# alibaba/TorchEasyRec

Measured on NVIDIA H100. Metric: samples/sec (DLRM-Criteo synth, train step fwd+bwd+optimizer), higher is better.
Workload: dtype f32

## Files before the change

torcheasyrec_b200/csrc/tzk_tower.cu:

```cuda
#include <cstdlib>

#include "tzk_common.cuh"

#include "tzk_launch.cuh"
#include "tzk_tower_bwd2.cuh"
#include "tzk_tower_tail.cuh"

using namespace tzk;

namespace {
constexpr int kTM = 128;

__device__ __forceinline__ int odd(int v) { return v | 1; }
constexpr int kNW = kTM / 32;
constexpr int kLU = 16;

__device__ __forceinline__ void load_tile(float* dst, int S, const float* __restrict__ src, int64_t ld,
                                          const float* __restrict__ mask, int64_t ld_m, int rows, int C) {
  const int warp = threadIdx.x >> 5, lane = threadIdx.x & 31;
  for (int r0 = warp; r0 < rows; r0 += kNW * kLU) {
    float v[kLU][2], m[kLU][2];
#pragma unroll
    for (int q = 0; q < kLU; ++q) {
      const int r = r0 + q * kNW;
// ... 262 lines not shown
  if ((threadIdx.x & 31) == 0) red[threadIdx.x >> 5] = acc;
  __syncthreads();
  if (threadIdx.x == 0) {
    float s = 0.f;
    for (int k = 0; k < kBceThreads / 32; ++k) s += red[k];
    partial[blockIdx.x] = s;
  }
}
__global__ void __launch_bounds__(256)
bce_final_kernel(const float* __restrict__ partial, int n, float inv_m, float* __restrict__ loss) {
  __shared__ float red[256];
  float s = 0.f;
  for (int i = threadIdx.x; i < n; i += 256) s += partial[i];
  red[threadIdx.x] = s;
  __syncthreads();
  for (int d = 128; d >= 1; d >>= 1) {
    if (threadIdx.x < d) red[threadIdx.x] += red[threadIdx.x + d];
    __syncthreads();
  }
  if (threadIdx.x == 0) loss[0] = red[0] * inv_m;
}
}

static int small_linear_check(const char* who, int64_t M, int32_t K, int32_t N) {
  TZK_REQUIRE(M >= 0, "%s: negative M", who);
  TZK_REQUIRE(K >= 1 && K <= 64 && N >= 1 && N <= 64, "%s: K=%d, N=%d outside [1,64]", who, K, N);
  return 0;
}

extern "C" int tzk_small_linear_fwd(const float* x, int64_t ld_x, const float* w, const float* bias, int64_t M,
                                    int32_t K, int32_t N, int32_t relu, float* y, int64_t ld_y,
                                    tzk_stream_t stream) {
  int rc = small_linear_check("small_linear_fwd", M, K, N);
  if (rc) return rc;
  if (M == 0) return 0;
  TZK_REQUIRE(x && w && y, "small_linear_fwd: NULL argument");
  TZK_REQUIRE(ld_x >= K && ld_y >= N, "small_linear_fwd: leading dimension smaller than the row");
  const int NP = pad_pow(N, 4);
  {
    const size_t smem_r = ((size_t)K * NP + NP) * sizeof(float);
    const bool vec = (K % 4 == 0) && (ld_x % 4 == 0) && ((uintptr_t)x % 16 == 0);
    const int64_t blocks = ceil_div64(M, kRowThreads);
    const int grid_r = (int)(blocks < kSmCountH100 * 16 ? blocks : kSmCountH100 * 16);
#define TZK_SLR(NP_)                                                                                                \
  do {                                                                                                              \
    if (vec)                                                                                                        \
      small_linear_fwd_rows_kernel<NP_, true><<<grid_r, kRowThreads, smem_r, as_stream(stream)>>>(                  \
          x, ld_x, w, bias, M, K, N, relu, y, ld_y);                                                                \
    else                                                                                                            \
      small_linear_fwd_rows_kernel<NP_, false><<<grid_r, kRowThreads, smem_r, as_stream(stream)>>>(                 \
          x, ld_x, w, bias, M, K, N, relu, y, ld_y);                                                                \
  } while (0)
    switch (NP) {
      case 4: TZK_SLR(4); break;
      case 16: TZK_SLR(16); break;
      case 32: TZK_SLR(32); break;
      default: TZK_SLR(64); break;
    }
#undef TZK_SLR
    TZK_CHECK_LAUNCH("small_linear_fwd_rows_kernel");
  }
  return 0;
}

static bool use_bwd2(int K, int N) {
  const char* e = getenv("TZK_SMALL_LINEAR_BWD");
  return !(e && e[0] == '1') && tzk_bwd2::supported(K, N);
}

extern "C" size_t tzk_small_linear_bwd_workspace_bytes(int64_t M, int32_t K, int32_t N) {
  const size_t v1 = (size_t)bwd_grid(M) * ((size_t)(N < 1 ? 1 : N) * (K < 1 ? 1 : K) + (N < 1 ? 1 : N)) * sizeof(float);
  const size_t v2 = tzk_bwd2::supported(K, N) ? tzk_bwd2::workspace_bytes(M < 1 ? 1 : M, K, N) : 0;
  return v1 > v2 ? v1 : v2;
}

extern "C" int tzk_small_linear_bwd(const float* x, int64_t ld_x, const float* w, const float* y, int64_t ld_y,
                                    const float* dy, int64_t ld_dy, int64_t M, int32_t K, int32_t N, int32_t relu,
                                    float* dx, int64_t ld_dx, float* dw, float* db, void* workspace,
                                    size_t workspace_bytes, tzk_stream_t stream) {
  int rc = small_linear_check("small_linear_bwd", M, K, N);
  if (rc) return rc;
  TZK_REQUIRE(M >= 1, "small_linear_bwd: empty batch");
  TZK_REQUIRE(x && w && dy && dw && (!relu || y), "small_linear_bwd: NULL argument");
  TZK_REQUIRE(ld_x >= K && ld_dy >= N && (!relu || ld_y >= N) && (!dx || ld_dx >= K),
              "small_linear_bwd: leading dimension smaller than the row");
  TZK_REQUIRE(workspace && workspace_bytes >= tzk_small_linear_bwd_workspace_bytes(M, K, N),
              "small_linear_bwd: workspace too small");
  if (use_bwd2(K, N)) {
    rc = tzk_bwd2::run(x, ld_x, w, y, ld_y, dy, ld_dy, M, K, N, relu, dx, ld_dx, dw, db, workspace, workspace_bytes,
                       as_stream(stream));
    TZK_REQUIRE(rc == 0, "small_linear_bwd: tzk_bwd2::run failed with code %d", rc);
    return 0;
  }
  const int KP = pad_pow(K, 16), NP = pad_pow(N, 4);
  const int grid = bwd_grid(M);
  const size_t smem = ((size_t)N * KP + (size_t)kTM * (K | 1) + (size_t)kTM * (N | 1)) * sizeof(float);
  float* partial = static_cast<float*>(workspace);
  cudaStream_t st = as_stream(stream);
#define TZK_SLB(KP_, NP_)                                                                                          \
  do {                                                                                                             \
    if (smem > 48 * 1024)                                                                                          \
      cudaFuncSetAttribute(small_linear_bwd_kernel<KP_, NP_>, cudaFuncAttributeMaxDynamicSharedMemorySize,         \
                           (int)smem);                                                                             \
    small_linear_bwd_kernel<KP_, NP_><<<grid, kTM, smem, st>>>(x, ld_x, w, y, ld_y, dy, ld_dy, M, K, N, relu, dx,   \
                                                               ld_dx, partial);                                    \
  } while (0)
#define TZK_SLB_N(KP_)                      \
  switch (NP) {                             \
    case 4: TZK_SLB(KP_, 4); break;         \
    case 16: TZK_SLB(KP_, 16); break;       \
    case 32: TZK_SLB(KP_, 32); break;       \
    default: TZK_SLB(KP_, 64); break;       \
  }
  switch (KP) {
    case 16: TZK_SLB_N(16) break;
    case 32: TZK_SLB_N(32) break;
    default: TZK_SLB_N(64) break;
  }
#undef TZK_SLB_N
#undef TZK_SLB
  TZK_CHECK_LAUNCH("small_linear_bwd_kernel");
  const int total = N * K + N;
  small_linear_reduce_kernel<<<(total + 31) / 32, 256, 0, st>>>(partial, grid, N * K, N, dw, db);
  TZK_CHECK_LAUNCH("small_linear_reduce_kernel");
  return 0;
}

extern "C" size_t tzk_bce_logits_workspace_bytes(int64_t M) {
  return (size_t)ceil_div64(M < 1 ? 1 : M, kBceThreads * kBcePerThread) * sizeof(float);
}

extern "C" int tzk_bce_logits_fwd_bwd(const float* logits, const float* labels, int64_t M, float* loss,
                                      float* dlogits, void* workspace, size_t workspace_bytes,
                                      tzk_stream_t stream) {
  TZK_REQUIRE(M >= 1, "bce_logits: empty batch");
  TZK_REQUIRE(logits && labels && loss, "bce_logits: NULL argument");
  TZK_REQUIRE(workspace && workspace_bytes >= tzk_bce_logits_workspace_bytes(M), "bce_logits: workspace too small");
  const int64_t nb = ceil_div64(M, kBceThreads * kBcePerThread);
  TZK_REQUIRE(nb < ((int64_t)1 << 31), "bce_logits: batch too large");
  float* partial = static_cast<float*>(workspace);
  cudaStream_t st = as_stream(stream);
  const float inv_m = 1.0f / (float)M;
  bce_fwd_bwd_kernel<<<(unsigned)nb, kBceThreads, 0, st>>>(logits, labels, M, inv_m, dlogits, partial);
  TZK_CHECK_LAUNCH("bce_fwd_bwd_kernel");
  bce_final_kernel<<<1, 256, 0, st>>>(partial, (int)nb, inv_m, loss);
  TZK_CHECK_LAUNCH("bce_final_kernel");
  return 0;
}

extern "C" size_t tzk_tower_tail_bce_workspace_bytes(int64_t M, int32_t K, int32_t N) {
  return tzk_tail::supported(K, N) ? tzk_tail::workspace_bytes(M < 1 ? 1 : M, K, N) : 0;
}

extern "C" int tzk_tower_tail_bce(const float* y1, int64_t ld_y, const float* w1, const float* b1, const float* w2,
                                  const float* b2, const float* labels, int64_t M, int32_t K, int32_t N, float* logits,
                                  float* dy1, int64_t ld_dy, float* colsum, float* out, void* workspace,
                                  size_t workspace_bytes, tzk_stream_t stream) {
  TZK_REQUIRE(M >= 1, "tower_tail_bce: empty batch");
  TZK_REQUIRE(tzk_tail::supported(K, N), "tower_tail_bce: K=%d, N=%d must be in [1, 64]", K, N);
  TZK_REQUIRE(y1 && w1 && w2 && labels && logits && dy1 && out, "tower_tail_bce: NULL argument");
  TZK_REQUIRE(ld_y >= K && ld_dy >= K, "tower_tail_bce: leading dimension smaller than the row");
  TZK_REQUIRE(workspace && workspace_bytes >= tzk_tower_tail_bce_workspace_bytes(M, K, N),
              "tower_tail_bce: workspace too small");
  const int rc = tzk_tail::run(y1, ld_y, w1, b1, w2, b2, labels, M, K, N, logits, dy1, ld_dy, out, workspace,
                               workspace_bytes, as_stream(stream), colsum != nullptr);
  TZK_REQUIRE(rc == 0, "tower_tail_bce: tzk_tail::run failed with code %d", rc);
  if (colsum) {
    colsum_final(static_cast<const float*>(workspace) + tzk_tail::colsum_offset(M, K, N), tzk_tail::tiles(M), K, colsum,
                 as_stream(stream));
    TZK_CHECK_LAUNCH("colsum_final_kernel");
  }
  return 0;
}
```

torcheasyrec_b200/csrc/tzk_tower_tail.cuh:

```cuda
#pragma once
#include <stdint.h>

namespace tzk_tail {
constexpr int kRows = 128;
constexpr int kMaxCtas = 132 * 4;

__device__ __forceinline__ bool aligned16(const void* p) { return (reinterpret_cast<uintptr_t>(p) & 15) == 0; }

inline int out_len(int K, int N) { return N * K + 2 * N + 2; }
inline int grid_for(int64_t M) {
  const int64_t t = (M + kRows - 1) / kRows;
  return (int)(t < 1 ? 1 : (t < kMaxCtas ? t : kMaxCtas));
}
inline int64_t tiles(int64_t M) { return (M + kRows - 1) / kRows; }
inline size_t colsum_offset(int64_t M, int K, int N) { return (size_t)grid_for(M) * out_len(K, N); }
inline size_t workspace_bytes(int64_t M, int K, int N) {
  return (colsum_offset(M, K, N) + (size_t)tiles(M) * K) * sizeof(float);
}
inline size_t smem_bytes(int KP, int NP, bool mask) {
  return ((size_t)NP * KP + 2 * NP + (size_t)(mask ? 2 : 1) * kRows * (KP + 4) + 2 * (size_t)kRows * NP + 2 * kRows) *
         sizeof(float);
}

template <int KP, int NP, bool kMask>
__global__ void __launch_bounds__(kRows)
tower_tail_bce_kernel(const float* __restrict__ y1, int64_t ld_y, const float* __restrict__ w1,
                      const float* __restrict__ b1, const float* __restrict__ w2, const float* __restrict__ b2,
                      const float* __restrict__ labels, int64_t M, int K, int N, float inv_m, int rows_per_cta,
                      float* __restrict__ logits, float* __restrict__ dy1, int64_t ld_dy, float* __restrict__ partial,
                      float* __restrict__ zsum) {
  constexpr int R = kRows, KC = KP / 4, NC = NP / 4, XS = KP + 4;
  constexpr int NB = (KC * NC + R - 1) / R;
  TZK_DYN_SMEM(float, sm);
  float* Ws = sm;
  float* b1s = Ws + NP * KP;
  float* w2s = b1s + NP;
  float* Xs = w2s + NP;
  float* Dh = Xs + R * XS;
  float* Hg = Dh + R * NP;
  float* Dz = Hg + R * NP;
  float* Ls = Dz + R;
  float* Zs = Ls + R;
  const int tid = threadIdx.x;
  for (int i = tid; i < NP * KP; i += R) {
    const int n = i / KP, k = i - n * KP;
    Ws[i] = (n < N && k < K) ? __ldg(w1 + (int64_t)n * K + k) : 0.f;
  }
  for (int n = tid; n < NP; n += R) {
    b1s[n] = (n < N && b1) ? __ldg(b1 + n) : 0.f;
    w2s[n] = n < N ? __ldg(w2 + n) : 0.f;
  }
  const float b2v = b2 ? __ldg(b2) : 0.f;
  const bool vin = (K & 3) == 0 && (ld_y & 3) == 0 && aligned16(y1);
  const bool vout = (K & 3) == 0 && (ld_dy & 3) == 0 && aligned16(dy1);
  float acc[NB][4][4], accv = 0.f, accw = 0.f, accz = 0.f, accl = 0.f;
#pragma unroll
  for (int q = 0; q < NB; ++q)
#pragma unroll
    for (int i = 0; i < 4; ++i)
#pragma unroll
      for (int j = 0; j < 4; ++j) acc[q][i][j] = 0.f;
  const int64_t row_begin = (int64_t)blockIdx.x * rows_per_cta;
  const int64_t row_end = row_begin + rows_per_cta < M ? row_begin + rows_per_cta : M;
  __syncthreads();
  for (int64_t t0 = row_begin; t0 < row_end; t0 += R) {
    const int64_t row = t0 + tid;
    const bool live = row < row_end;
    float* xr = Xs + tid * XS;
#pragma unroll
    for (int c = 0; c < KC; ++c) {
      float4 v = make_float4(0.f, 0.f, 0.f, 0.f);
      if (live && 4 * c < K) {
        const float* p = y1 + row * ld_y + 4 * c;
        if (vin) {
          v = *reinterpret_cast<const float4*>(p);
        } else {
          v.x = __ldg(p);
          if (4 * c + 1 < K) v.y = __ldg(p + 1);
          if (4 * c + 2 < K) v.z = __ldg(p + 2);
          if (4 * c + 3 < K) v.w = __ldg(p + 3);
        }
      }
      *reinterpret_cast<float4*>(xr + 4 * c) = v;
    }
    float h[NP];
#pragma unroll
    for (int n = 0; n < NP; ++n) h[n] = b1s[n];
#pragma unroll 2
    for (int c = 0; c < KC; ++c) {
      const float4 x4 = *reinterpret_cast<const float4*>(xr + 4 * c);
#pragma unroll
      for (int n = 0; n < NP; ++n) {
        const float4 w4 = *reinterpret_cast<const float4*>(Ws + n * KP + 4 * c);
        h[n] = fmaf(x4.x, w4.x, h[n]);
        h[n] = fmaf(x4.y, w4.y, h[n]);
        h[n] = fmaf(x4.z, w4.z, h[n]);
        h[n] = fmaf(x4.w, w4.w, h[n]);
      }
    }
    float z = b2v;
#pragma unroll
    for (int n = 0; n < NP; ++n) {
      h[n] = h[n] > 0.f ? h[n] : 0.f;
      z = fmaf(h[n], w2s[n], z);
    }
    float dz = 0.f, lt = 0.f;
    if (live) {
      const float y = __ldg(labels + row);
      const float e = expf(-fabsf(z));
      lt = fmaxf(z, 0.f) - z * y + log1pf(e);
      const float sig = z >= 0.f ? 1.f / (1.f + e) : e / (1.f + e);
      dz = (sig - y) * inv_m;
      logits[row] = z;
    }
    Dz[tid] = dz;
    Ls[tid] = lt;
#pragma unroll
    for (int n = 0; n < NP; ++n) {
      Hg[tid * NP + n] = dz * h[n];
      h[n] = h[n] > 0.f ? dz * w2s[n] : 0.f;
      Dh[tid * NP + n] = h[n];
    }
#pragma unroll 2
    for (int c = 0; c < KC; ++c) {
      float4 a = make_float4(0.f, 0.f, 0.f, 0.f);
#pragma unroll
      for (int n = 0; n < NP; ++n) {
        const float4 w4 = *reinterpret_cast<const float4*>(Ws + n * KP + 4 * c);
        a.x = fmaf(h[n], w4.x, a.x);
        a.y = fmaf(h[n], w4.y, a.y);
        a.z = fmaf(h[n], w4.z, a.z);
        a.w = fmaf(h[n], w4.w, a.w);
      }
      if constexpr (kMask) {
        const float4 y4 = *reinterpret_cast<const float4*>(xr + 4 * c);
        a.x = y4.x > 0.f ? a.x : 0.f;
        a.y = y4.y > 0.f ? a.y : 0.f;
        a.z = y4.z > 0.f ? a.z : 0.f;
        a.w = y4.w > 0.f ? a.w : 0.f;
        *reinterpret_cast<float4*>(Zs + tid * XS + 4 * c) = a;
      }
      if (live && 4 * c < K) {
        float* p = dy1 + row * ld_dy + 4 * c;
        if (vout) {
          *reinterpret_cast<float4*>(p) = a;
        } else {
          p[0] = a.x;
          if (4 * c + 1 < K) p[1] = a.y;
          if (4 * c + 2 < K) p[2] = a.z;
          if (4 * c + 3 < K) p[3] = a.w;
        }
      }
    }
    __syncthreads();
#pragma unroll
    for (int q = 0; q < NB; ++q) {
      const int blk = tid + q * R;
      if (blk < KC * NC) {
        const int tn = blk / KC, tk = blk - tn * KC;
        const float* dp = Dh + 4 * tn;
        const float* xp = Xs + 4 * tk;
#pragma unroll 4
        for (int r = 0; r < R; ++r) {
          const float4 a4 = *reinterpret_cast<const float4*>(dp + r * NP);
          const float4 b4 = *reinterpret_cast<const float4*>(xp + r * XS);
          const float a[4] = {a4.x, a4.y, a4.z, a4.w}, b[4] = {b4.x, b4.y, b4.z, b4.w};
#pragma unroll
          for (int i = 0; i < 4; ++i)
#pragma unroll
            for (int j = 0; j < 4; ++j) acc[q][i][j] = fmaf(a[i], b[j], acc[q][i][j]);
        }
      }
    }
    if (tid < NP) {
      for (int r = 0; r < R; ++r) {
        accv += Dh[r * NP + tid];
        accw += Hg[r * NP + tid];
      }
    }
    if (tid == 0) {
      for (int r = 0; r < R; ++r) {
        accz += Dz[r];
        accl += Ls[r];
      }
    }
    if constexpr (kMask) {
      const int c = tid - (R - KP);
      if (c >= 0 && c < K) {
        float s[4] = {0.f, 0.f, 0.f, 0.f};
#pragma unroll 4
        for (int r = 0; r < R; r += 4)
#pragma unroll
          for (int j = 0; j < 4; ++j) s[j] += Zs[(r + j) * XS + c];
        float v = 0.f;
#pragma unroll
        for (int j = 0; j < 4; ++j) v += s[j];
        zsum[t0 / R * K + c] = v;
      }
    }
    __syncthreads();
  }
  float* out = partial + (int64_t)blockIdx.x * (N * K + 2 * N + 2);
#pragma unroll
  for (int q = 0; q < NB; ++q) {
    const int blk = tid + q * R;
    if (blk < KC * NC) {
      const int tn = blk / KC, tk = blk - tn * KC;
#pragma unroll
      for (int i = 0; i < 4; ++i)
#pragma unroll
        for (int j = 0; j < 4; ++j)
          if (4 * tn + i < N && 4 * tk + j < K) out[(4 * tn + i) * K + 4 * tk + j] = acc[q][i][j];
    }
  }
  if (tid < N) {
    out[N * K + tid] = accv;
    out[N * K + N + tid] = accw;
  }
  if (tid == 0) {
    out[N * K + 2 * N] = accz;
    out[N * K + 2 * N + 1] = accl;
  }
}

__global__ void __launch_bounds__(256)
tower_tail_reduce_kernel(const float* __restrict__ partial, int n_parts, int len, float inv_m, float* __restrict__ out) {
  __shared__ float red[8][32];
  const int o = threadIdx.x & 31, g = threadIdx.x >> 5;
  const int i = blockIdx.x * 32 + o;
  float s = 0.f;
  if (i < len)
    for (int c = g; c < n_parts; c += 8) s += partial[(int64_t)c * len + i];
  red[g][o] = s;
  __syncthreads();
  if (g == 0 && i < len) {
    float r = 0.f;
#pragma unroll
    for (int k = 0; k < 8; ++k) r += red[k][o];
    out[i] = i == len - 1 ? r * inv_m : r;
  }
}

inline bool supported(int K, int N) { return K >= 1 && N >= 1 && K <= 64 && N <= 64; }

inline int run(const float* y1, int64_t ld_y, const float* w1, const float* b1, const float* w2, const float* b2,
               const float* labels, int64_t M, int32_t K, int32_t N, float* logits, float* dy1, int64_t ld_dy,
               float* out, void* workspace, size_t workspace_bytes_, cudaStream_t st, bool mask = false) {
  if (M < 1 || !supported(K, N) || !y1 || !w1 || !w2 || !labels || !logits || !dy1 || !out || ld_y < K || ld_dy < K) return 1;
  if (workspace_bytes_ < workspace_bytes(M, K, N)) return 2;
  const int KP = K <= 16 ? 16 : (K <= 32 ? 32 : 64);
  const int NP = N <= 16 ? 16 : (N <= 32 ? 32 : 64);
  const int grid = grid_for(M);
  int rows_per_cta = (int)((M + grid - 1) / grid);
  rows_per_cta = (rows_per_cta + kRows - 1) / kRows * kRows;
  const float inv_m = 1.0f / (float)M;
  const size_t smem = smem_bytes(KP, NP, mask);
  float* partial = static_cast<float*>(workspace);
  float* zsum = partial + colsum_offset(M, K, N);
#ifdef TZK_CPU_SHIM
#define TZK_TAIL_ATTR(KP_, NP_, MASK_)
#else
#define TZK_TAIL_ATTR(KP_, NP_, MASK_)                                                                                \
  if (smem > 48 * 1024)                                                                                               \
    cudaFuncSetAttribute(tower_tail_bce_kernel<KP_, NP_, MASK_>, cudaFuncAttributeMaxDynamicSharedMemorySize, (int)smem);
#endif
#define TZK_TAIL(KP_, NP_, MASK_)                                                                                     \
  do {                                                                                                                \
    TZK_TAIL_ATTR(KP_, NP_, MASK_)                                                                                    \
    TZK_LAUNCH((tower_tail_bce_kernel<KP_, NP_, MASK_>), grid, kRows, smem, st, y1, ld_y, w1, b1, w2, b2, labels, M,  \
               K, N, inv_m, rows_per_cta, logits, dy1, ld_dy, partial, zsum);                                         \
  } while (0)
#define TZK_TAIL_N(KP_, MASK_)                                                                                        \
  do {                                                                                                                \
    if (NP == 16) TZK_TAIL(KP_, 16, MASK_);                                                                           \
    else if (NP == 32) TZK_TAIL(KP_, 32, MASK_);                                                                      \
    else TZK_TAIL(KP_, 64, MASK_);                                                                                    \
  } while (0)
#define TZK_TAIL_K(MASK_)                                                                                             \
  do {                                                                                                                \
    if (KP == 16) TZK_TAIL_N(16, MASK_);                                                                              \
    else if (KP == 32) TZK_TAIL_N(32, MASK_);                                                                         \
    else TZK_TAIL_N(64, MASK_);                                                                                       \
  } while (0)
  if (mask) TZK_TAIL_K(true);
  else TZK_TAIL_K(false);
#undef TZK_TAIL_K
#undef TZK_TAIL_N
#undef TZK_TAIL
#undef TZK_TAIL_ATTR
  if (cudaGetLastError() != cudaSuccess) return 3;
  const int len = out_len(K, N);
  TZK_LAUNCH((tower_tail_reduce_kernel), (len + 31) / 32, 256, 0, st, partial, grid, len, inv_m, out);
  return cudaGetLastError() == cudaSuccess ? 0 : 3;
}
}
```

torcheasyrec_b200/kernels.py:

```python

import ctypes
import math
import os
import threading
from dataclasses import dataclass
from typing import List, Optional, Sequence, Tuple

import torch

from ._lib import TzkError, check, lib

POOL_SUM, POOL_MEAN = 0, 1
OPT_SGD, OPT_ADAGRAD, OPT_ROWWISE_ADAGRAD, OPT_ADAM, OPT_PARTIAL_ROWWISE_ADAM = 0, 1, 2, 3, 4
OPT_LAMB, OPT_PARTIAL_ROWWISE_LAMB, OPT_LARS_SGD = 5, 6, 7
WD_NONE, WD_L2, WD_DECOUPLE = 0, 1, 2
LARS_ETA = 0.001
OPT_ACCUM_OUT = 100


@dataclass
class FeatureLayout:

    w_off: List[int]
    rows: List[int]
# ... 794 lines not shown
        d_sparse = torch.empty((B, 416), dtype=torch.float32, device=sparse.device)
        check(self._lib.tzk_dot_interact27_bwd_bf16(_ptr(d_out), ld_o, _ptr(dense), ld_d, _ptr(sparse), ld_s, B,
                                                    _ptr(d_dense), 16, _ptr(d_sparse), 416, _stream()),
              "tzk_dot_interact27_bwd_bf16")
        self.launches += 1
        return d_dense, d_sparse

    def interact_wide_fwd(self, dense: torch.Tensor, sparse: torch.Tensor, w: torch.Tensor, bias: Optional[torch.Tensor]):
        dense, ld_d = _rows2d(dense, "dense")
        sparse, ld_s = _rows2d(sparse, "sparse")
        w, ld_w = _rows2d(w, "w")
        B = dense.shape[0]
        y = torch.empty((B, 64), dtype=torch.float32, device=dense.device)
        pairs = torch.empty((B, 352), dtype=torch.float32, device=dense.device)
        ws = torch.empty((2, 64, 784), dtype=torch.float32, device=dense.device)
        check(self._lib.tzk_interact_wide_fwd(_ptr(dense), ld_d, _ptr(sparse), ld_s, _ptr(w), ld_w, _ptr(bias), B,
                                              _ptr(y), 64, _ptr(pairs), 352, _ptr(ws[0]), _ptr(ws[1]), _stream()),
              "tzk_interact_wide_fwd")
        self.launches += 2
        return y, pairs

    def interact_wide_wgrad(self, dz: torch.Tensor, pairs: torch.Tensor, dense: torch.Tensor, sparse: torch.Tensor,
                            slabs: int, scale: Optional[torch.Tensor] = None) -> torch.Tensor:
        dz, ld_z = _rows2d(dz, "dz")
        pairs, ld_p = _rows2d(pairs, "pairs")
        dense, ld_d = _rows2d(dense, "dense")
        sparse, ld_s = _rows2d(sparse, "sparse")
        B = dz.shape[0]
        dw = torch.empty((64, 784), dtype=torch.float32, device=dz.device)
        part = torch.empty(slabs * 896 * 64, dtype=torch.float32, device=dz.device)
        if scale is not None and _need(scale, torch.float32, "scale").numel() != 1:
            raise TzkError("scale: expected one element")
        check(self._lib.tzk_interact_wide_wgrad_scaled(_ptr(dz), ld_z, _ptr(scale), _ptr(pairs), ld_p, _ptr(dense), ld_d,
                                                       _ptr(sparse), ld_s, B, slabs, _ptr(part), _ptr(dw), 784,
                                                       _stream()), "tzk_interact_wide_wgrad_scaled")
        self.launches += 2
        return dw

    def interact_wide_bwd(self, dz: torch.Tensor, w: torch.Tensor, dense: torch.Tensor, sparse: torch.Tensor,
                          scale: Optional[torch.Tensor] = None):
        dz, ld_z = _rows2d(dz, "dz")
        w, ld_w = _rows2d(w, "w")
        dense, ld_d = _rows2d(dense, "dense")
        sparse, ld_s = _rows2d(sparse, "sparse")
        B = dz.shape[0]
        d_dense = torch.empty((B, 16), dtype=torch.float32, device=dz.device)
        d_sparse = torch.empty((B, 416), dtype=torch.float32, device=dz.device)
        wt = torch.empty((2, 784, 64), dtype=torch.float32, device=dz.device)
        if scale is not None and _need(scale, torch.float32, "scale").numel() != 1:
            raise TzkError("scale: expected one element")
        check(self._lib.tzk_interact_wide_bwd_scaled(_ptr(dz), ld_z, _ptr(scale), _ptr(w), ld_w, _ptr(dense), ld_d,
                                                     _ptr(sparse), ld_s, B, _ptr(d_dense), 16, _ptr(d_sparse), 416,
                                                     _ptr(wt[0]), _ptr(wt[1]), _stream()),
              "tzk_interact_wide_bwd_scaled")
        self.launches += 2
        return d_dense, d_sparse

    def bias_act(self, y: torch.Tensor, bias: Optional[torch.Tensor], relu: bool) -> torch.Tensor:
        y, ld = _rows2d(y, "y")
        check(self._lib.tzk_bias_act(_ptr(y), ld, _ptr(bias), y.shape[0], y.shape[1], int(relu), _stream()),
              "tzk_bias_act")
        self.launches += 1
        return y

    def act_bwd_colsum(self, dy: torch.Tensor, y: Optional[torch.Tensor], relu: bool, want_dz: bool = True,
                       out: Optional[torch.Tensor] = None):
        dy, ld_dy = _rows2d(dy, "dy")
        M, N = dy.shape
        ld_y = 0
        if y is not None:
            y, ld_y = _rows2d(y, "y")
        if out is not None:
            dz, ld_dz = _rows2d(out, "out")
        else:
            dz, ld_dz = (torch.empty((M, N), dtype=torch.float32, device=dy.device) if want_dz else None), N
        colsum = torch.empty(N, dtype=torch.float32, device=dy.device)
        nb = self._lib.tzk_act_bwd_colsum_workspace_bytes(M, N)
        ws = self._workspace("colsum", nb, dy.device)
        check(self._lib.tzk_act_bwd_colsum(_ptr(dy), ld_dy, _ptr(y), ld_y, M, N, int(relu), _ptr(dz), ld_dz,
                                           _ptr(colsum), _ptr(ws), ws.numel(), _stream()), "tzk_act_bwd_colsum")
        self.launches += 2
        return dz, colsum
    def small_linear_fwd(self, x: torch.Tensor, w: torch.Tensor, bias: Optional[torch.Tensor],
                         relu: bool) -> torch.Tensor:
        x, ld_x = _rows2d(x, "x")
        _need(w, torch.float32, "w")
        M, K = x.shape
        N = w.shape[0]
        if w.shape[1] != K:
            raise TzkError(f"small_linear_fwd: x has {K} columns, w expects {w.shape[1]}")
        y = torch.empty((M, N), dtype=torch.float32, device=x.device)
        if M:
            check(self._lib.tzk_small_linear_fwd(_ptr(x), ld_x, _ptr(w), _ptr(bias), M, K, N, int(relu), _ptr(y), N,
                                                 _stream()), "tzk_small_linear_fwd")
            self.launches += 1
        return y

    def small_linear_bwd(self, x: torch.Tensor, w: torch.Tensor, y: Optional[torch.Tensor], dy: torch.Tensor,
                         relu: bool, want_dx: bool, want_db: bool):
        x, ld_x = _rows2d(x, "x")
        dy, ld_dy = _rows2d(dy, "dy")
        _need(w, torch.float32, "w")
        M, K = x.shape
        N = w.shape[0]
        ld_y = 0
        if relu:
            y, ld_y = _rows2d(y, "y")
        dx = torch.empty((M, K), dtype=torch.float32, device=x.device) if want_dx else None
        dw = torch.empty((N, K), dtype=torch.float32, device=x.device)
        db = torch.empty(N, dtype=torch.float32, device=x.device) if want_db else None
        nb = self._lib.tzk_small_linear_bwd_workspace_bytes(M, K, N)
        ws = self._workspace(("slb", K, N), nb, x.device)
        check(self._lib.tzk_small_linear_bwd(_ptr(x), ld_x, _ptr(w), _ptr(y) if relu else None, ld_y, _ptr(dy), ld_dy,
                                             M, K, N, int(relu), _ptr(dx), K, _ptr(dw), _ptr(db), _ptr(ws),
                                             ws.numel(), _stream()), "tzk_small_linear_bwd")
        self.launches += (2 + int(want_dx)) if _small_linear_rows_path(K, N) else 2
        return dx, dw, db

    def bce_logits_fwd_bwd(self, logits: torch.Tensor, labels: torch.Tensor, want_grad: bool = True):
        _need(logits, torch.float32, "logits")
        _need(labels, torch.float32, "labels")
        M = logits.numel()
        if labels.numel() != M:
            raise TzkError("bce_logits: logits and labels differ in size")
        loss = torch.empty((), dtype=torch.float32, device=logits.device)
        dz = torch.empty(M, dtype=torch.float32, device=logits.device) if want_grad else None
        nb = self._lib.tzk_bce_logits_workspace_bytes(M)
        ws = self._workspace("bce", nb, logits.device)
        check(self._lib.tzk_bce_logits_fwd_bwd(_ptr(logits), _ptr(labels), M, _ptr(loss), _ptr(dz), _ptr(ws),
                                               ws.numel(), _stream()), "tzk_bce_logits_fwd_bwd")
        self.launches += 2
        return loss, dz

    def tower_tail_bce(self, y1: torch.Tensor, w1: torch.Tensor, b1: Optional[torch.Tensor], w2: torch.Tensor,
                       b2: Optional[torch.Tensor], labels: torch.Tensor, relu_dz: bool = False):
        y1, ld = _rows2d(y1, "y1")
        _need(w1, torch.float32, "w1")
        _need(w2, torch.float32, "w2")
        _need(labels, torch.float32, "labels")
        M, K = y1.shape
        N = w1.shape[0]
        if w1.shape != (N, K) or w2.numel() != N or labels.numel() != M:
            raise TzkError("tower_tail_bce: shapes do not chain")
        dev = y1.device
        logits = torch.empty(M, dtype=torch.float32, device=dev)
        dy1 = torch.empty((M, K), dtype=torch.float32, device=dev)
        out = torch.empty(N * K + 2 * N + 2, dtype=torch.float32, device=dev)
        colsum = torch.empty(K, dtype=torch.float32, device=dev) if relu_dz else None
        nb = self._lib.tzk_tower_tail_bce_workspace_bytes(M, K, N)
        ws = self._workspace("tail", nb, dev)
        check(self._lib.tzk_tower_tail_bce(_ptr(y1), ld, _ptr(w1), _ptr(b1), _ptr(w2), _ptr(b2), _ptr(labels), M, K, N,
                                           _ptr(logits), _ptr(dy1), K, _ptr(colsum), _ptr(out), _ptr(ws), ws.numel(),
                                           _stream()), "tzk_tower_tail_bce")
        self.launches += 3 if relu_dz else 2
        o = N * K
        return (out[o + 2 * N + 1], logits, dy1, out[:o].view(N, K), out[o:o + N], out[o + N:o + 2 * N].view(1, N),
                out[o + 2 * N:o + 2 * N + 1], colsum)

    def binned_auc_update(self, preds: torch.Tensor, labels: torch.Tensor, thresholds: torch.Tensor,
                          counts: torch.Tensor, invalid: torch.Tensor) -> None:
        if preds.dtype not in (torch.float32, torch.bfloat16):
            raise TzkError(f"binned_auc_update: predictions must be float32 or bfloat16, got {preds.dtype}")
        if labels.dtype not in (torch.float32, torch.int64):
            raise TzkError(f"binned_auc_update: labels must be float32 or int64, got {labels.dtype}")
        _need(preds, preds.dtype, "preds")
        _need(labels, labels.dtype, "labels")
        _need(thresholds, torch.float32, "thresholds")
        _need(counts, torch.int64, "counts")
        _need(invalid, torch.int64, "invalid")
        n, T = preds.numel(), thresholds.numel()
        if labels.numel() != n:
            raise TzkError(f"binned_auc_update: {n} predictions but {labels.numel()} labels")
        if T < 1 or counts.numel() != 2 * (T + 1) or invalid.numel() != 1:
            raise TzkError("binned_auc_update: counts must be [T + 1, 2] and invalid [1] for T >= 1 thresholds")
        check(self._lib.tzk_binned_auc_update(_ptr(preds), int(preds.dtype == torch.bfloat16), _ptr(labels),
                                              int(labels.dtype == torch.int64), n, _ptr(thresholds), T, _ptr(counts),
                                              _ptr(invalid), _stream()), "tzk_binned_auc_update")
        self.launches += int(n > 0)

    def _grid(self, work: int, per_sm: int, slices: int = 1) -> int:
        sms = getattr(self, "_sms", None)
        if sms is None:
            sms = self._sms = max(1, int(self._lib.tzk_sm_count()))
        return max(1, min(int(work), -(-per_sm * sms // slices)))

    def _batch_sums(self, key: str, grid: int, shapes, device):
        sizes = [math.prod(s) for s in shapes]
        partials = self._workspace(key, grid * sum(sizes) * 4, device)
        dparams = torch.empty(sum(sizes), dtype=torch.float32, device=device)
        return partials, dparams, [v.view(s) for v, s in zip(dparams.split(sizes), shapes)]

    def wukong_mix_fwd(self, x, w_fmb, gamma, beta, w_lcb, w_res, f: int):
        for t, nm in ((x, "x"), (w_fmb, "w_fmb"), (gamma, "gamma"), (beta, "beta"), (w_lcb, "w_lcb")):
            _need(t, torch.float32, nm)
        if w_res is not None:
            _need(w_res, torch.float32, "w_res")
        B, n, d = x.shape
        k, l = w_fmb.shape[1], w_lcb.shape[1]
        m = f + l
        ln_f = torch.empty((B, n * k), dtype=torch.float32, device=x.device)
        stats = torch.empty((B, 2), dtype=torch.float32, device=x.device)
        base = torch.empty((B, m, d), dtype=torch.float32, device=x.device)
        check(self._lib.tzk_wukong_mix_fwd(_ptr(x), _ptr(w_fmb), _ptr(gamma), _ptr(beta), _ptr(w_lcb), _ptr(w_res), B,
                                           n, d, k, f, l, self._grid(B, 8), _ptr(ln_f), _ptr(stats), _ptr(base),
                                           _stream()), "tzk_wukong_mix_fwd")
        self.launches += int(B > 0)
        return ln_f, stats, base

    def wukong_mix_bwd(self, x, w_fmb, gamma, w_lcb, w_res, f: int, stats, d_ln_f, d_base):
        for t, nm in ((x, "x"), (w_fmb, "w_fmb"), (gamma, "gamma"), (w_lcb, "w_lcb"), (stats, "stats"),
                      (d_ln_f, "d_ln_f"), (d_base, "d_base")):
            _need(t, torch.float32, nm)
        if w_res is not None:
            _need(w_res, torch.float32, "w_res")
        B, n, d = x.shape
        k, l = w_fmb.shape[1], w_lcb.shape[1]
        m = f + l
        grid = self._grid(B, 4)
        dx = torch.empty_like(x)
        partials, dparams, (dw_fmb, dw_lcb, dw_res, dgamma, dbeta) = self._batch_sums(
            "wukong_mix_bwd", grid, [(n, k), (n, l), (n, m if w_res is not None else 0), (n * k,), (n * k,)], x.device)
        check(self._lib.tzk_wukong_mix_bwd(_ptr(x), _ptr(w_fmb), _ptr(gamma), _ptr(w_lcb), _ptr(w_res), _ptr(stats),
                                           _ptr(d_ln_f), _ptr(d_base), B, n, d, k, f, l, grid, _ptr(dx),
                                           _ptr(partials), _ptr(dparams), _stream()), "tzk_wukong_mix_bwd")
        self.launches += 1 + int(B > 0)
        return dx, dw_fmb, dgamma, dbeta, dw_lcb, (dw_res if w_res is not None else None)

    def wukong_out_fwd(self, fmb_out, base, gamma, beta, f: int):
        for t, nm in ((fmb_out, "fmb_out"), (base, "base"), (gamma, "gamma"), (beta, "beta")):
            _need(t, torch.float32, nm)
        B, m, d = base.shape
        y = torch.empty_like(base)
        stats = torch.empty((B, m, 2), dtype=torch.float32, device=base.device)
        check(self._lib.tzk_wukong_out_fwd(_ptr(fmb_out), _ptr(base), _ptr(gamma), _ptr(beta), B, d, f, m - f,
                                           self._grid(-(-B * m // 128), 8), _ptr(y), _ptr(stats), _stream()),
              "tzk_wukong_out_fwd")
        self.launches += int(B > 0)
        return y, stats

    def wukong_out_bwd(self, fmb_out, base, gamma, f: int, stats, dy):
        for t, nm in ((fmb_out, "fmb_out"), (base, "base"), (gamma, "gamma"), (stats, "stats"), (dy, "dy")):
            _need(t, torch.float32, nm)
        B, m, d = base.shape
        grid = self._grid(-(-B * m // 128), 4)
        d_fmb = torch.empty_like(fmb_out)
        d_base = torch.empty_like(base)
        partials, dparams, (dgamma, dbeta) = self._batch_sums("wukong_out_bwd", grid, [(d,), (d,)], base.device)
        check(self._lib.tzk_wukong_out_bwd(_ptr(fmb_out), _ptr(base), _ptr(gamma), _ptr(stats), _ptr(dy), B, d, f,
                                           m - f, grid, _ptr(d_fmb), _ptr(d_base), _ptr(partials), _ptr(dparams),
                                           _stream()), "tzk_wukong_out_bwd")
        self.launches += 1 + int(B > 0)
        return d_fmb, d_base, dgamma, dbeta


    def masknet_mask_fwd(self, e, m, b2, gamma, beta, E: int, nb: int):
        for t, nm in ((e, "e"), (m, "m"), (b2, "b2"), (gamma, "gamma"), (beta, "beta")):
            _need(t, torch.float32, nm)
        B = e.shape[0]
        v = torch.empty_like(m)
        stats = torch.empty((B, 2), dtype=torch.float32, device=e.device)
        check(self._lib.tzk_masknet_mask_fwd(_ptr(e), e.shape[1], _ptr(m), _ptr(b2), _ptr(gamma), _ptr(beta), B, E, nb,
                                             self._grid(B, 8), _ptr(v), _ptr(stats), _stream()),
              "tzk_masknet_mask_fwd")
        self.launches += int(B > 0)
        return v, stats

    def masknet_mask_bwd(self, e, m, b2, gamma, beta, stats, dv, E: int, nb: int):
        for t, nm in ((e, "e"), (m, "m"), (b2, "b2"), (gamma, "gamma"), (beta, "beta"), (stats, "stats"),
                      (dv, "dv")):
            _need(t, torch.float32, nm)
        B = e.shape[0]
        grid = self._grid(B, 6)
        dm = torch.empty_like(m)
        de = torch.empty_like(e)
        partials, dparams, (db2, dgamma, dbeta) = self._batch_sums("masknet_mask_bwd", grid, [(nb * E,), (E,), (E,)],
                                                                   e.device)
        check(self._lib.tzk_masknet_mask_bwd(_ptr(e), e.shape[1], _ptr(m), _ptr(b2), _ptr(gamma), _ptr(beta),
                                             _ptr(stats), _ptr(dv), B, E, nb, grid, _ptr(dm), _ptr(de),
                                             _ptr(partials), _ptr(dparams), _stream()), "tzk_masknet_mask_bwd")
        self.launches += 1 + int(B > 0)
        return dm, de, db2, dgamma, dbeta

    def masknet_ffn_fwd(self, z, b3, gamma, beta, nb: int):
        for t, nm in ((z, "z"), (b3, "b3"), (gamma, "gamma"), (beta, "beta")):
            _need(t, torch.float32, nm)
        B, H = z.shape[0], z.shape[1] // nb
        y = torch.empty_like(z)
        stats = torch.empty((B, nb, 2), dtype=torch.float32, device=z.device)
        check(self._lib.tzk_masknet_ffn_fwd(_ptr(z), _ptr(b3), _ptr(gamma), _ptr(beta), B, H, nb,
                                            self._grid(B, 6, nb), _ptr(y), _ptr(stats), _stream()),
              "tzk_masknet_ffn_fwd")
        self.launches += int(B > 0)
        return y, stats

    def masknet_ffn_bwd(self, z, b3, gamma, beta, stats, dy, nb: int):
        for t, nm in ((z, "z"), (b3, "b3"), (gamma, "gamma"), (beta, "beta"), (stats, "stats"), (dy, "dy")):
            _need(t, torch.float32, nm)
        B, H = z.shape[0], z.shape[1] // nb
        grid = self._grid(B, 5, nb)
        dz = torch.empty_like(z)
        partials, dparams, (g3,) = self._batch_sums("masknet_ffn_bwd", grid, [(nb, 3, H)], z.device)
        check(self._lib.tzk_masknet_ffn_bwd(_ptr(z), _ptr(b3), _ptr(gamma), _ptr(beta), _ptr(stats), _ptr(dy), B, H,
                                            nb, grid, _ptr(dz), _ptr(partials), _ptr(dparams), _stream()),
              "tzk_masknet_ffn_bwd")
        self.launches += 1 + int(B > 0)
        return dz, g3[:, 0], g3[:, 1], g3[:, 2]

# ... 358 lines not shown
```

Measured before the change: 54.94 million.

## Restructure tower tail kernel: coalesced tile loads, smaller smem, fused colsum reduce

Rewrites the fused tower-tail BCE kernel so each CTA loads its 128-row input tile cooperatively with coalesced float4 loads and writes dy1 back coalesced from shared memory, instead of one thread per row striding through global memory. The Dh/Hg/Zs buffers are merged into a single padded Ds buffer that is reused across phases, and the per-column reductions are spread across threads. Shared memory drops and launch bounds now request 2-3 CTAs per SM. The separate colsum_final launch is folded into the tail reduce kernel. An optional globaltimer instrumentation path sits behind a compile flag. The cost is extra __syncthreads per tile.

```diff
diff --git a/torcheasyrec_b200/csrc/tzk_tower.cu b/torcheasyrec_b200/csrc/tzk_tower.cu
--- a/torcheasyrec_b200/csrc/tzk_tower.cu
+++ b/torcheasyrec_b200/csrc/tzk_tower.cu
@@ -438,6 +438,12 @@
   return tzk_tail::supported(K, N) ? tzk_tail::workspace_bytes(M < 1 ? 1 : M, K, N) : 0;
 }
 
+#ifdef TZK_TAIL_TIMING
+extern "C" int tzk_tower_tail_timing(unsigned long long* buf) {
+  return cudaMemcpyToSymbol(tzk_tail::tail_timing, &buf, sizeof(buf)) == cudaSuccess ? 0 : 1;
+}
+#endif
+
 extern "C" int tzk_tower_tail_bce(const float* y1, int64_t ld_y, const float* w1, const float* b1, const float* w2,
                                   const float* b2, const float* labels, int64_t M, int32_t K, int32_t N, float* logits,
                                   float* dy1, int64_t ld_dy, float* colsum, float* out, void* workspace,
@@ -449,12 +455,7 @@
   TZK_REQUIRE(workspace && workspace_bytes >= tzk_tower_tail_bce_workspace_bytes(M, K, N),
               "tower_tail_bce: workspace too small");
   const int rc = tzk_tail::run(y1, ld_y, w1, b1, w2, b2, labels, M, K, N, logits, dy1, ld_dy, out, workspace,
-                               workspace_bytes, as_stream(stream), colsum != nullptr);
+                               workspace_bytes, as_stream(stream), colsum != nullptr, colsum);
   TZK_REQUIRE(rc == 0, "tower_tail_bce: tzk_tail::run failed with code %d", rc);
-  if (colsum) {
-    colsum_final(static_cast<const float*>(workspace) + tzk_tail::colsum_offset(M, K, N), tzk_tail::tiles(M), K, colsum,
-                 as_stream(stream));
-    TZK_CHECK_LAUNCH("colsum_final_kernel");
-  }
   return 0;
 }
diff --git a/torcheasyrec_b200/csrc/tzk_tower_tail.cuh b/torcheasyrec_b200/csrc/tzk_tower_tail.cuh
--- a/torcheasyrec_b200/csrc/tzk_tower_tail.cuh
+++ b/torcheasyrec_b200/csrc/tzk_tower_tail.cuh
@@ -3,44 +3,58 @@
 
 namespace tzk_tail {
 constexpr int kRows = 128;
-constexpr int kMaxCtas = 132 * 4;
+constexpr int kMaxSegs = 132 * 4;
 
 __device__ __forceinline__ bool aligned16(const void* p) { return (reinterpret_cast<uintptr_t>(p) & 15) == 0; }
 
+#ifdef TZK_TAIL_TIMING
+__device__ unsigned long long* tail_timing;
+__device__ __forceinline__ unsigned long long tail_now() {
+  unsigned long long t;
+  asm volatile("mov.u64 %0, %%globaltimer;" : "=l"(t));
+  return t;
+}
+#define TAIL_STAMP(tile, slot) do { if (threadIdx.x == 0) tail_timing[4 * (tile) + (slot)] = tail_now(); } while (0)
+#else
+#define TAIL_STAMP(tile, slot) do {} while (0)
+#endif
+
 inline int out_len(int K, int N) { return N * K + 2 * N + 2; }
-inline int grid_for(int64_t M) {
-  const int64_t t = (M + kRows - 1) / kRows;
-  return (int)(t < 1 ? 1 : (t < kMaxCtas ? t : kMaxCtas));
-}
 inline int64_t tiles(int64_t M) { return (M + kRows - 1) / kRows; }
-inline size_t colsum_offset(int64_t M, int K, int N) { return (size_t)grid_for(M) * out_len(K, N); }
+inline int segments(int64_t M) {
+  const int64_t t = tiles(M);
+  return (int)(t < 1 ? 1 : (t < kMaxSegs ? t : kMaxSegs));
+}
+inline int rows_per_segment(int64_t M) {
+  const int s = segments(M);
+  const int64_t r = (M + s - 1) / s;
+  return (int)((r + kRows - 1) / kRows * kRows);
+}
+inline size_t colsum_offset(int64_t M, int K, int N) { return (size_t)segments(M) * out_len(K, N); }
 inline size_t workspace_bytes(int64_t M, int K, int N) {
   return (colsum_offset(M, K, N) + (size_t)tiles(M) * K) * sizeof(float);
 }
-inline size_t smem_bytes(int KP, int NP, bool mask) {
-  return ((size_t)NP * KP + 2 * NP + (size_t)(mask ? 2 : 1) * kRows * (KP + 4) + 2 * (size_t)kRows * NP + 2 * kRows) *
-         sizeof(float);
+inline size_t smem_bytes(int KP, int NP) {
+  return ((size_t)NP * KP + 2 * NP + (size_t)kRows * (KP + 4) + (size_t)kRows * (NP + 4) + 2 * kRows) * sizeof(float);
 }
 
 template <int KP, int NP, bool kMask>
-__global__ void __launch_bounds__(kRows)
+__global__ void __launch_bounds__(kRows, KP == 64 && NP <= 32 ? 3 : 2)
 tower_tail_bce_kernel(const float* __restrict__ y1, int64_t ld_y, const float* __restrict__ w1,
                       const float* __restrict__ b1, const float* __restrict__ w2, const float* __restrict__ b2,
-                      const float* __restrict__ labels, int64_t M, int K, int N, float inv_m, int rows_per_cta,
-                      float* __restrict__ logits, float* __restrict__ dy1, int64_t ld_dy, float* __restrict__ partial,
-                      float* __restrict__ zsum) {
-  constexpr int R = kRows, KC = KP / 4, NC = NP / 4, XS = KP + 4;
+                      const float* __restrict__ labels, int64_t M, int K, int N, float inv_m, int rows_per_seg,
+                      float* __restrict__ logits, float* __restrict__ dy1, int64_t ld_dy,
+                      float* __restrict__ partial, float* __restrict__ zsum) {
+  constexpr int R = kRows, KC = KP / 4, NC = NP / 4, XS = KP + 4, NS = NP + 4;
   constexpr int NB = (KC * NC + R - 1) / R;
   TZK_DYN_SMEM(float, sm);
   float* Ws = sm;
   float* b1s = Ws + NP * KP;
   float* w2s = b1s + NP;
   float* Xs = w2s + NP;
-  float* Dh = Xs + R * XS;
-  float* Hg = Dh + R * NP;
-  float* Dz = Hg + R * NP;
+  float* Ds = Xs + R * XS;
+  float* Dz = Ds + R * NS;
   float* Ls = Dz + R;
-  float* Zs = Ls + R;
   const int tid = threadIdx.x;
   for (int i = tid; i < NP * KP; i += R) {
     const int n = i / KP, k = i - n * KP;
@@ -53,191 +67,210 @@
   const float b2v = b2 ? __ldg(b2) : 0.f;
   const bool vin = (K & 3) == 0 && (ld_y & 3) == 0 && aligned16(y1);
   const bool vout = (K & 3) == 0 && (ld_dy & 3) == 0 && aligned16(dy1);
-  float acc[NB][4][4], accv = 0.f, accw = 0.f, accz = 0.f, accl = 0.f;
-#pragma unroll
-  for (int q = 0; q < NB; ++q)
-#pragma unroll
-    for (int i = 0; i < 4; ++i)
-#pragma unroll
-      for (int j = 0; j < 4; ++j) acc[q][i][j] = 0.f;
-  const int64_t row_begin = (int64_t)blockIdx.x * rows_per_cta;
-  const int64_t row_end = row_begin + rows_per_cta < M ? row_begin + rows_per_cta : M;
+  const int nw = tid - (R - NP), cz = tid;
+  const float* sec = nw == 1 ? Ls : Dz;
+  float* xr = Xs + tid * XS;
+  float* dr = Ds + tid * NS;
   __syncthreads();
-  for (int64_t t0 = row_begin; t0 < row_end; t0 += R) {
-    const int64_t row = t0 + tid;
-    const bool live = row < row_end;
-    float* xr = Xs + tid * XS;
-#pragma unroll
-    for (int c = 0; c < KC; ++c) {
-      float4 v = make_float4(0.f, 0.f, 0.f, 0.f);
-      if (live && 4 * c < K) {
-        const float* p = y1 + row * ld_y + 4 * c;
-        if (vin) {
-          v = *reinterpret_cast<const float4*>(p);
-        } else {
-          v.x = __ldg(p);
-          if (4 * c + 1 < K) v.y = __ldg(p + 1);
-          if (4 * c + 2 < K) v.z = __ldg(p + 2);
-          if (4 * c + 3 < K) v.w = __ldg(p + 3);
-        }
-      }
-      *reinterpret_cast<float4*>(xr + 4 * c) = v;
+  {
+    const int seg = blockIdx.x;
+    float acc[NB][4][4], accv[NB], accw = 0.f, acc2 = 0.f;
+#pragma unroll
+    for (int q = 0; q < NB; ++q) {
+      accv[q] = 0.f;
+#pragma unroll
+      for (int i = 0; i < 4; ++i)
+#pragma unroll
+        for (int j = 0; j < 4; ++j) acc[q][i][j] = 0.f;
     }
-    float h[NP];
-#pragma unroll
-    for (int n = 0; n < NP; ++n) h[n] = b1s[n];
+    const int64_t row_begin = (int64_t)seg * rows_per_seg;
+    const int64_t row_end = row_begin + rows_per_seg < M ? row_begin + rows_per_seg : M;
+    for (int64_t t0 = row_begin; t0 < row_end; t0 += R) {
+      TAIL_STAMP(t0 / R, 0);
+      const int64_t row = t0 + tid;
+      const bool live = row < row_end;
+      const int64_t live_rows = row_end - t0 < R ? row_end - t0 : R;
+      if (vin) {
+#pragma unroll 8
+        for (int j = 0; j < KC; ++j) {
+          const int i = tid + j * R, r = i / KC, c = i - r * KC;
+          float4 v = make_float4(0.f, 0.f, 0.f, 0.f);
+          if (r < live_rows && 4 * c < K) v = *reinterpret_cast<const float4*>(y1 + (t0 + r) * ld_y + 4 * c);
+          *reinterpret_cast<float4*>(Xs + r * XS + 4 * c) = v;
+        }
+      } else {
+        for (int i = tid; i < R * KP; i += R) {
+          const int r = i / KP, k = i - r * KP;
+          Xs[r * XS + k] = (r < live_rows && k < K) ? __ldg(y1 + (t0 + r) * ld_y + k) : 0.f;
+        }
+      }
+      __syncthreads();
+      float h[NP];
+#pragma unroll
+      for (int n = 0; n < NP; ++n) h[n] = b1s[n];
 #pragma unroll 2
-    for (int c = 0; c < KC; ++c) {
-      const float4 x4 = *reinterpret_cast<const float4*>(xr + 4 * c);
+      for (int c = 0; c < KC; ++c) {
+        const float4 x4 = *reinterpret_cast<const float4*>(xr + 4 * c);
+#pragma unroll
+        for (int n = 0; n < NP; ++n) {
+          const float4 w4 = *reinterpret_cast<const float4*>(Ws + n * KP + 4 * c);
+          h[n] = fmaf(x4.x, w4.x, h[n]);
+          h[n] = fmaf(x4.y, w4.y, h[n]);
+          h[n] = fmaf(x4.z, w4.z, h[n]);
+          h[n] = fmaf(x4.w, w4.w, h[n]);
+        }
+      }
+      float z = b2v;
 #pragma unroll
       for (int n = 0; n < NP; ++n) {
-        const float4 w4 = *reinterpret_cast<const float4*>(Ws + n * KP + 4 * c);
-        h[n] = fmaf(x4.x, w4.x, h[n]);
-        h[n] = fmaf(x4.y, w4.y, h[n]);
-        h[n] = fmaf(x4.z, w4.z, h[n]);
-        h[n] = fmaf(x4.w, w4.w, h[n]);
-      }
+        h[n] = h[n] > 0.f ? h[n] : 0.f;
+        z = fmaf(h[n], w2s[n], z);
+      }
+      float dz = 0.f, lt = 0.f;
+      if (live) {
+        const float y = __ldg(labels + row);
+        const float e = expf(-fabsf(z));
+        lt = fmaxf(z, 0.f) - z * y + log1pf(e);
+        const float sig = z >= 0.f ? 1.f / (1.f + e) : e / (1.f + e);
+        dz = (sig - y) * inv_m;
+        logits[row] = z;
+      }
+      Dz[tid] = dz;
+      Ls[tid] = lt;
+#pragma unroll
+      for (int n = 0; n < NP; n += 4)
+        *reinterpret_cast<float4*>(dr + n) =
+            make_float4(h[n] > 0.f ? dz * w2s[n] : 0.f, h[n + 1] > 0.f ? dz * w2s[n + 1] : 0.f,
+                        h[n + 2] > 0.f ? dz * w2s[n + 2] : 0.f, h[n + 3] > 0.f ? dz * w2s[n + 3] : 0.f);
+      __syncthreads();
+      TAIL_STAMP(t0 / R, 1);
+#pragma unroll
+      for (int q = 0; q < NB; ++q) {
+        const int blk = tid + q * R;
+        if (blk < KC * NC) {
+          const int tn = blk / KC, tk = blk - tn * KC;
+          const float* dp = Ds + 4 * tn;
+          const float* xp = Xs + 4 * tk;
+#pragma unroll 4
+          for (int r = 0; r < R; ++r) {
+            const float4 a4 = *reinterpret_cast<const float4*>(dp + r * NS);
+            const float4 b4 = *reinterpret_cast<const float4*>(xp + r * XS);
+            const float a[4] = {a4.x, a4.y, a4.z, a4.w}, b[4] = {b4.x, b4.y, b4.z, b4.w};
+#pragma unroll
+            for (int i = 0; i < 4; ++i)
+#pragma unroll
+              for (int j = 0; j < 4; ++j) acc[q][i][j] = fmaf(a[i], b[j], acc[q][i][j]);
+            accv[q] += tk == 0 ? a4.x : tk == 1 ? a4.y : tk == 2 ? a4.z : a4.w;
+          }
+        }
+      }
+      __syncthreads();
+#pragma unroll
+      for (int n = 0; n < NP; n += 4) {
+        *reinterpret_cast<float4*>(dr + n) = make_float4(dz * h[n], dz * h[n + 1], dz * h[n + 2], dz * h[n + 3]);
+#pragma unroll
+        for (int i = n; i < n + 4; ++i) h[i] = h[i] > 0.f ? dz * w2s[i] : 0.f;
+      }
+#pragma unroll 2
+      for (int c = 0; c < KC; ++c) {
+        float4 a = make_float4(0.f, 0.f, 0.f, 0.f);
+#pragma unroll
+        for (int n = 0; n < NP; ++n) {
+          const float4 w4 = *reinterpret_cast<const float4*>(Ws + n * KP + 4 * c);
+          a.x = fmaf(h[n], w4.x, a.x);
+          a.y = fmaf(h[n], w4.y, a.y);
+          a.z = fmaf(h[n], w4.z, a.z);
+          a.w = fmaf(h[n], w4.w, a.w);
+        }
+        if constexpr (kMask) {
+          const float4 y4 = *reinterpret_cast<const float4*>(xr + 4 * c);
+          a.x = y4.x > 0.f ? a.x : 0.f;
+          a.y = y4.y > 0.f ? a.y : 0.f;
+          a.z = y4.z > 0.f ? a.z : 0.f;
+          a.w = y4.w > 0.f ? a.w : 0.f;
+        }
+        *reinterpret_cast<float4*>(xr + 4 * c) = a;
+      }
+      __syncthreads();
+      TAIL_STAMP(t0 / R, 2);
+      if (vout) {
+#pragma unroll 8
+        for (int j = 0; j < KC; ++j) {
+          const int i = tid + j * R, r = i / KC, c = i - r * KC;
+          if (r < live_rows && 4 * c < K)
+            *reinterpret_cast<float4*>(dy1 + (t0 + r) * ld_dy + 4 * c) = *reinterpret_cast<const float4*>(Xs + r * XS + 4 * c);
+        }
+      } else {
+        for (int i = tid; i < R * KP; i += R) {
+          const int r = i / KP, k = i - r * KP;
+          if (r < live_rows && k < K) dy1[(t0 + r) * ld_dy + k] = Xs[r * XS + k];
+        }
+      }
+      if (nw >= 0) {
+#pragma unroll 8
+        for (int r = 0; r < R; ++r) {
+          accw += Ds[r * NS + nw];
+          acc2 += sec[r];
+        }
+      }
+      if constexpr (kMask) {
+        if (cz < K) {
+          float s[4] = {0.f, 0.f, 0.f, 0.f};
+#pragma unroll 8
+          for (int r = 0; r < R; r += 4)
+#pragma unroll
+            for (int j = 0; j < 4; ++j) s[j] += Xs[(r + j) * XS + cz];
+          float v = 0.f;
+#pragma unroll
+          for (int j = 0; j < 4; ++j) v += s[j];
+          zsum[t0 / R * K + cz] = v;
+        }
+      }
+      __syncthreads();
+      TAIL_STAMP(t0 / R, 3);
     }
-    float z = b2v;
-#pragma unroll
-    for (int n = 0; n < NP; ++n) {
-      h[n] = h[n] > 0.f ? h[n] : 0.f;
-      z = fmaf(h[n], w2s[n], z);
-    }
-    float dz = 0.f, lt = 0.f;
-    if (live) {
-      const float y = __ldg(labels + row);
-      const float e = expf(-fabsf(z));
-      lt = fmaxf(z, 0.f) - z * y + log1pf(e);
-      const float sig = z >= 0.f ? 1.f / (1.f + e) : e / (1.f + e);
-      dz = (sig - y) * inv_m;
-      logits[row] = z;
-    }
-    Dz[tid] = dz;
-    Ls[tid] = lt;
-#pragma unroll
-    for (int n = 0; n < NP; ++n) {
-      Hg[tid * NP + n] = dz * h[n];
-      h[n] = h[n] > 0.f ? dz * w2s[n] : 0.f;
-      Dh[tid * NP + n] = h[n];
-    }
-#pragma unroll 2
-    for (int c = 0; c < KC; ++c) {
-      float4 a = make_float4(0.f, 0.f, 0.f, 0.f);
-#pragma unroll
-      for (int n = 0; n < NP; ++n) {
-        const float4 w4 = *reinterpret_cast<const float4*>(Ws + n * KP + 4 * c);
-        a.x = fmaf(h[n], w4.x, a.x);
-        a.y = fmaf(h[n], w4.y, a.y);
-        a.z = fmaf(h[n], w4.z, a.z);
-        a.w = fmaf(h[n], w4.w, a.w);
-      }
-      if constexpr (kMask) {
-        const float4 y4 = *reinterpret_cast<const float4*>(xr + 4 * c);
-        a.x = y4.x > 0.f ? a.x : 0.f;
-        a.y = y4.y > 0.f ? a.y : 0.f;
-        a.z = y4.z > 0.f ? a.z : 0.f;
-        a.w = y4.w > 0.f ? a.w : 0.f;
-        *reinterpret_cast<float4*>(Zs + tid * XS + 4 * c) = a;
-      }
-      if (live && 4 * c < K) {
-        float* p = dy1 + row * ld_dy + 4 * c;
-        if (vout) {
-          *reinterpret_cast<float4*>(p) = a;
-        } else {
-          p[0] = a.x;
-          if (4 * c + 1 < K) p[1] = a.y;
-          if (4 * c + 2 < K) p[2] = a.z;
-          if (4 * c + 3 < K) p[3] = a.w;
-        }
-      }
-    }
-    __syncthreads();
+    float* out = partial + (int64_t)seg * (N * K + 2 * N + 2);
 #pragma unroll
     for (int q = 0; q < NB; ++q) {
       const int blk = tid + q * R;
       if (blk < KC * NC) {
         const int tn = blk / KC, tk = blk - tn * KC;
-        const float* dp = Dh + 4 * tn;
-        const float* xp = Xs + 4 * tk;
-#pragma unroll 4
-        for (int r = 0; r < R; ++r) {
-          const float4 a4 = *reinterpret_cast<const float4*>(dp + r * NP);
-          const float4 b4 = *reinterpret_cast<const float4*>(xp + r * XS);
-          const float a[4] = {a4.x, a4.y, a4.z, a4.w}, b[4] = {b4.x, b4.y, b4.z, b4.w};
-#pragma unroll
-          for (int i = 0; i < 4; ++i)
-#pragma unroll
-            for (int j = 0; j < 4; ++j) acc[q][i][j] = fmaf(a[i], b[j], acc[q][i][j]);
-        }
+#pragma unroll
+        for (int i = 0; i < 4; ++i)
+#pragma unroll
+          for (int j = 0; j < 4; ++j)
+            if (4 * tn + i < N && 4 * tk + j < K) out[(4 * tn + i) * K + 4 * tk + j] = acc[q][i][j];
+        if (tk < 4 && 4 * tn + tk < N) out[N * K + 4 * tn + tk] = accv[q];
       }
     }
-    if (tid < NP) {
-      for (int r = 0; r < R; ++r) {
-        accv += Dh[r * NP + tid];
-        accw += Hg[r * NP + tid];
-      }
-    }
-    if (tid == 0) {
-      for (int r = 0; r < R; ++r) {
-        accz += Dz[r];
-        accl += Ls[r];
-      }
-    }
-    if constexpr (kMask) {
-      const int c = tid - (R - KP);
-      if (c >= 0 && c < K) {
-        float s[4] = {0.f, 0.f, 0.f, 0.f};
-#pragma unroll 4
-        for (int r = 0; r < R; r += 4)
-#pragma unroll
-          for (int j = 0; j < 4; ++j) s[j] += Zs[(r + j) * XS + c];
-        float v = 0.f;
-#pragma unroll
-        for (int j = 0; j < 4; ++j) v += s[j];
-        zsum[t0 / R * K + c] = v;
-      }
-    }
-    __syncthreads();
-  }
-  float* out = partial + (int64_t)blockIdx.x * (N * K + 2 * N + 2);
-#pragma unroll
-  for (int q = 0; q < NB; ++q) {
-    const int blk = tid + q * R;
-    if (blk < KC * NC) {
-      const int tn = blk / KC, tk = blk - tn * KC;
-#pragma unroll
-      for (int i = 0; i < 4; ++i)
-#pragma unroll
-        for (int j = 0; j < 4; ++j)
-          if (4 * tn + i < N && 4 * tk + j < K) out[(4 * tn + i) * K + 4 * tk + j] = acc[q][i][j];
-    }
-  }
-  if (tid < N) {
-    out[N * K + tid] = accv;
-    out[N * K + N + tid] = accw;
-  }
-  if (tid == 0) {
-    out[N * K + 2 * N] = accz;
-    out[N * K + 2 * N + 1] = accl;
+    if (nw >= 0 && nw < N) out[N * K + N + nw] = accw;
+    if (nw == 0 || nw == 1) out[N * K + 2 * N + nw] = acc2;
   }
 }
 
 __global__ void __launch_bounds__(256)
-tower_tail_reduce_kernel(const float* __restrict__ partial, int n_parts, int len, float inv_m, float* __restrict__ out) {
+tower_tail_reduce_kernel(const float* __restrict__ partial, int n_parts, int len, float inv_m, float* __restrict__ out,
+                         const float* __restrict__ zsum, int n_tiles, int K, float* __restrict__ colsum) {
   __shared__ float red[8][32];
   const int o = threadIdx.x & 31, g = threadIdx.x >> 5;
-  const int i = blockIdx.x * 32 + o;
+  const int out_blocks = (len + 31) / 32;
+  const bool cols = (int)blockIdx.x >= out_blocks;
+  const float* src = cols ? zsum : partial;
+  const int n = cols ? n_tiles : n_parts, w = cols ? K : len;
+  const int i = (cols ? (int)blockIdx.x - out_blocks : (int)blockIdx.x) * 32 + o;
   float s = 0.f;
-  if (i < len)
-    for (int c = g; c < n_parts; c += 8) s += partial[(int64_t)c * len + i];
+  if (i < w) {
+#pragma unroll 8
+    for (int c = g; c < n; c += 8) s += src[(int64_t)c * w + i];
+  }
   red[g][o] = s;
   __syncthreads();
-  if (g == 0 && i < len) {
+  if (g == 0 && i < w) {
     float r = 0.f;
 #pragma unroll
     for (int k = 0; k < 8; ++k) r += red[k][o];
-    out[i] = i == len - 1 ? r * inv_m : r;
+    if (cols) colsum[i] = r;
+    else out[i] = i == len - 1 ? r * inv_m : r;
   }
 }
 
@@ -245,16 +278,15 @@
 
 inline int run(const float* y1, int64_t ld_y, const float* w1, const float* b1, const float* w2, const float* b2,
                const float* labels, int64_t M, int32_t K, int32_t N, float* logits, float* dy1, int64_t ld_dy,
-               float* out, void* workspace, size_t workspace_bytes_, cudaStream_t st, bool mask = false) {
+               float* out, void* workspace, size_t workspace_bytes_, cudaStream_t st, bool mask = false,
+               float* colsum = nullptr) {
   if (M < 1 || !supported(K, N) || !y1 || !w1 || !w2 || !labels || !logits || !dy1 || !out || ld_y < K || ld_dy < K) return 1;
   if (workspace_bytes_ < workspace_bytes(M, K, N)) return 2;
   const int KP = K <= 16 ? 16 : (K <= 32 ? 32 : 64);
   const int NP = N <= 16 ? 16 : (N <= 32 ? 32 : 64);
-  const int grid = grid_for(M);
-  int rows_per_cta = (int)((M + grid - 1) / grid);
-  rows_per_cta = (rows_per_cta + kRows - 1) / kRows * kRows;
+  const int n_seg = segments(M), rows_per_seg = rows_per_segment(M);
   const float inv_m = 1.0f / (float)M;
-  const size_t smem = smem_bytes(KP, NP, mask);
+  const size_t smem = smem_bytes(KP, NP);
   float* partial = static_cast<float*>(workspace);
   float* zsum = partial + colsum_offset(M, K, N);
 #ifdef TZK_CPU_SHIM
@@ -267,8 +299,8 @@
 #define TZK_TAIL(KP_, NP_, MASK_)                                                                                     \
   do {                                                                                                                \
     TZK_TAIL_ATTR(KP_, NP_, MASK_)                                                                                    \
-    TZK_LAUNCH((tower_tail_bce_kernel<KP_, NP_, MASK_>), grid, kRows, smem, st, y1, ld_y, w1, b1, w2, b2, labels, M,  \
-               K, N, inv_m, rows_per_cta, logits, dy1, ld_dy, partial, zsum);                                         \
+    TZK_LAUNCH((tower_tail_bce_kernel<KP_, NP_, MASK_>), n_seg, kRows, smem, st, y1, ld_y, w1, b1, w2, b2, labels,    \
+               M, K, N, inv_m, rows_per_seg, logits, dy1, ld_dy, partial, zsum);                                      \
   } while (0)
 #define TZK_TAIL_N(KP_, MASK_)                                                                                        \
   do {                                                                                                                \
@@ -290,7 +322,9 @@
 #undef TZK_TAIL_ATTR
   if (cudaGetLastError() != cudaSuccess) return 3;
   const int len = out_len(K, N);
-  TZK_LAUNCH((tower_tail_reduce_kernel), (len + 31) / 32, 256, 0, st, partial, grid, len, inv_m, out);
+  const bool cols = mask && colsum;
+  TZK_LAUNCH((tower_tail_reduce_kernel), (len + 31) / 32 + (cols ? (K + 31) / 32 : 0), 256, 0, st, partial, n_seg,
+             len, inv_m, out, zsum, (int)tiles(M), K, colsum);
   return cudaGetLastError() == cudaSuccess ? 0 : 3;
 }
 }
diff --git a/torcheasyrec_b200/kernels.py b/torcheasyrec_b200/kernels.py
--- a/torcheasyrec_b200/kernels.py
+++ b/torcheasyrec_b200/kernels.py
@@ -970,7 +970,7 @@
         check(self._lib.tzk_tower_tail_bce(_ptr(y1), ld, _ptr(w1), _ptr(b1), _ptr(w2), _ptr(b2), _ptr(labels), M, K, N,
                                            _ptr(logits), _ptr(dy1), K, _ptr(colsum), _ptr(out), _ptr(ws), ws.numel(),
                                            _stream()), "tzk_tower_tail_bce")
-        self.launches += 3 if relu_dz else 2
+        self.launches += 2
         o = N * K
         return (out[o + 2 * N + 1], logits, dy1, out[:o].view(N, K), out[o:o + N], out[o + N:o + 2 * N].view(1, N),
                 out[o + 2 * N:o + 2 * N + 1], colsum)
```

Measured after the change: 56.09 million, median of 6. 2.1% higher.
